# zsc/MOSS-TTSD

Measured on AMD Instinct MI355X. Metric: audio codec tokens/sec/node (decode, bf16, batch 32 @ 4k ctx), higher is better.
Workload: dtype bf16; 1 GPU; configs[2]: batch 32 synthetic dialogues/GPU, 4k-token KV context, top-k/top-p sampling on 8 channels, decode steps at full context; batch_per_gpu=32, context=4096, prompt=512, layers=28, hidden=2048, parallelism=dp1 (batch shard, no per-step collective)

## Files before the change

### moss-ttsd_amd/csrc/attn.hip

```cpp
#include "launch.h"
#include <algorithm>
#include <atomic>
#include <cstdlib>
#ifndef MTTS_PK_WAVES
#define MTTS_PK_WAVES 0
#endif
#if MTTS_PK_WAVES
#define PK_OCC(PK) __attribute__((amdgpu_waves_per_eu((PK) ? MTTS_PK_WAVES : 1, (PK) ? MTTS_PK_WAVES : 8)))
#else
#define PK_OCC(PK)
#endif

#include "seal.h"

__device__ bool seal_lane_k(const u32x4_t* __restrict__ raw, u32x4_t* __restrict__ pk, uint8_t* __restrict__ lds, int lane) {
    u32x4_t v[16];
#pragma unroll
    for (int j = 0; j < 16; ++j) v[j] = raw[j * 64];
    __builtin_amdgcn_wave_barrier();
    uint32_t* row = (uint32_t*)(lds + lane * 128);
#pragma unroll
    for (int j = 0; j < 16; ++j)
#pragma unroll
        for (int c = 0; c < 4; c += 2) {
// ... 128 lines not shown
    if (r < R) m = meta[r];
    unsigned long long todo = __ballot(m.seq >= 0 && (m.pos & 63) == 63);
    while (todo) {
        const int i = __ffsll((long long)todo) - 1;
        todo &= todo - 1;
        const int seq = __shfl(m.seq, i, 64), pos = __shfl(m.pos, i, 64);
        const int page = page_table[(size_t)seq * max_pages + (pos >> 6)];
        const size_t pi = (size_t)kvh * total_pages + page;
        const bool fit = wave ? seal_lane_v(vcache + layer * raw_layer + pi * (MTTS_PAGE * MTTS_HD / 8) + lane,
                                            vpack + layer * pk_layer + pi * (MTTS_PKU * 64) + lane, vlds, lane)
                              : seal_lane_k(kcache + layer * raw_layer + pi * (MTTS_PAGE * MTTS_HD / 8) + lane,
                                            kpack + layer * pk_layer + pi * (MTTS_PKU * 64) + lane, klds, lane);
        seal_count(fit, cnt, layer, wave, lane);
    }
}
__global__ __launch_bounds__(128) void kv_seal_all_kernel(const u32x4_t* __restrict__ kcache, const u32x4_t* __restrict__ vcache,
                                                          u32x4_t* __restrict__ kpack, u32x4_t* __restrict__ vpack, int total_pages,
                                                          size_t raw_layer, size_t pk_layer, unsigned long long* __restrict__ cnt) {
    __shared__ __attribute__((aligned(16))) uint8_t klds[8192 + 128];
    __shared__ __attribute__((aligned(16))) uint8_t vlds[8192 + 320];
    const int kvh = blockIdx.y, layer = blockIdx.z, wave = threadIdx.x >> 6, lane = threadIdx.x & 63;
    const size_t pi = (size_t)kvh * total_pages + blockIdx.x;
    const bool fit = wave ? seal_lane_v(vcache + layer * raw_layer + pi * (MTTS_PAGE * MTTS_HD / 8) + lane,
                                        vpack + layer * pk_layer + pi * (MTTS_PKU * 64) + lane, vlds, lane)
                          : seal_lane_k(kcache + layer * raw_layer + pi * (MTTS_PAGE * MTTS_HD / 8) + lane,
                                        kpack + layer * pk_layer + pi * (MTTS_PKU * 64) + lane, klds, lane);
    seal_count(fit, cnt, layer, wave, lane);
}
__global__ __launch_bounds__(64) void kv_seal_pages_kernel(const u32x4_t* __restrict__ raw, u32x4_t* __restrict__ pk, int as_k) {
    __shared__ __attribute__((aligned(16))) uint8_t klds[8192 + 320];
// ... 18 lines not shown
        n += 1;
        dk += __any(fk.w != 0u) ? 1 : 0;
        dv += __any(fv.w != 0u) ? 1 : 0;
    }
    if (lane == 0 && n) {
        atomicAdd(out + 0, n); atomicAdd(out + 1, dk); atomicAdd(out + 2, n); atomicAdd(out + 3, dv);
    }
}
void launch_kv_pack_count(const void* kpack, const void* vpack, const int32_t* page_table, const int32_t* complete, int B, int max_pages,
                          int total_pages, int nkv, int L, unsigned long long* out, hipStream_t st) {
    const size_t pk_layer = (size_t)total_pages * nkv * (MTTS_PKU * 64);
    hipLaunchKernelGGL(kv_pack_count_kernel, dim3(B, nkv, L), dim3(64), 0, st, (const u32x4_t*)kpack, (const u32x4_t*)vpack, page_table,
                       complete, max_pages, total_pages, pk_layer, out);
}
void launch_kv_seal_rows(const void* kcache, const void* vcache, void* kpack, void* vpack, const int32_t* page_table,
                         const RowMeta* meta, int R, int max_pages, int total_pages, int nkv, int L, unsigned long long* cnt, hipStream_t st) {
    const size_t raw_layer = (size_t)total_pages * nkv * (MTTS_PAGE * MTTS_HD / 8), pk_layer = (size_t)total_pages * nkv * (MTTS_PKU * 64);
    hipLaunchKernelGGL(kv_seal_scan_kernel, dim3((R + 63) / 64, nkv, L), dim3(128), 0, st, (const u32x4_t*)kcache, (const u32x4_t*)vcache,
                       (u32x4_t*)kpack, (u32x4_t*)vpack, page_table, meta, R, max_pages, total_pages, raw_layer, pk_layer, cnt);
}
void launch_kv_seal_all(const void* kcache, const void* vcache, void* kpack, void* vpack, int total_pages, int nkv, int L,
                        unsigned long long* cnt, hipStream_t st) {
    const size_t raw_layer = (size_t)total_pages * nkv * (MTTS_PAGE * MTTS_HD / 8), pk_layer = (size_t)total_pages * nkv * (MTTS_PKU * 64);
    hipLaunchKernelGGL(kv_seal_all_kernel, dim3(total_pages, nkv, L), dim3(128), 0, st, (const u32x4_t*)kcache, (const u32x4_t*)vcache,
                       (u32x4_t*)kpack, (u32x4_t*)vpack, total_pages, raw_layer, pk_layer, cnt);
}


__device__ __forceinline__ void fuse_reduce(const QkvFuse& f, int r, int col, int lane, float& a, float& b) {
    const size_t kstride = (size_t)MTTS_PFCAP * f.Npad;
    const float* p0 = f.partial + (size_t)r * f.Npad + col + lane;
    a = 0.f; b = 0.f;
    for (int k0 = 0; k0 < f.ksplit; k0 += 8) {
// ... 1068 lines not shown
```

### moss-ttsd_amd/csrc/engine.h

```cpp
#pragma once
#include <hip/hip_runtime.h>

#include <algorithm>
#include <cstdarg>
#include <cstdio>
#include <cstdlib>
#include <cstring>
#include <memory>
#include <string>
#include <vector>

#include "launch.h"
#include "runstate.h"
#include "stepplan.h"

static_assert(RUN_EINVAL == MTTS_EINVAL, "runstate.h reports with MTTS_EINVAL");

#define MTTS_LOCAL __attribute__((visibility("hidden")))
extern MTTS_LOCAL thread_local char g_err[512];
#define HIPCHK(x)                                                                          \
    do {                                                                                   \
        hipError_t _e = (x);                                                               \
        if (_e != hipSuccess) return fail(MTTS_EHIP, "%s: %s (%s:%d)", #x, hipGetErrorString(_e), __FILE__, __LINE__); \
    } while (0)
// ... 192 lines not shown

static inline bool rows_carry_adapters(const MttsEngine* e) {
    for (int b = 0; b < e->B; ++b)
        if (e->seq_adapter[b] >= 0) return true;
    return false;
}
static inline StepState step_state(const MttsEngine* e, int heads, int R, int pages_bound, bool lora) {
    StepState s;
    s.heads = heads; s.B = e->B; s.R = R; s.pages_bound = pages_bound; s.lora = lora;
    s.forced = e->has_forced; s.ch0_sampled = e->ch0_sampled != 0; s.scores_on = e->scores_on != 0; s.floors_on = e->floors_on != 0;
    s.bans_on = e->bans_on != 0;
    s.topk = e->topk_on;
    for (int k = 0; k < WSEAL_KINDS; ++k) s.wseal_on[k] = e->wseal_on[k] != 0;
    if (e->kpack) s.pack_k_on = e->pack_k_on.data();
    if (e->vpack) s.pack_v_on = e->pack_v_on.data();
    return s;
}
static inline StepPlan decode_plan(const MttsEngine* e, int pages_bound) {
    return plan_step(e->knobs, e->caps, step_state(e, 1, round_up(e->B, 32), pages_bound, rows_carry_adapters(e)));
}

static inline KvPack layer_pack(const MttsEngine* e, const StepPlan& plan, int n) {
    const LayerPlan& l = plan.layers[n];
    return KvPack{l.k_sealed ? (uint8_t*)e->kpack + e->pk_layer_stride * n : nullptr,
                  l.v_sealed ? (uint8_t*)e->vpack + e->pk_layer_stride * n : nullptr};
}
```

### moss-ttsd_amd/csrc/engine.hip

```cpp
#include "engine.h"
#include "staging.h"

#define FLUSH_STEPS 7
#define LINGER_STEPS 14
static inline int linger_bound(int B) { return 6 * B + 8; }

thread_local char g_err[512] = "";
int fail(int code, const char* fmt, ...) {
    va_list ap;
    va_start(ap, fmt);
    vsnprintf(g_err, sizeof(g_err), fmt, ap);
    va_end(ap);
    return code;
}

const char* mtts_last_error(void) { return g_err; }
int32_t mtts_version(void) { return 202; }

static auto ship_on(MttsEngine* e, hipStream_t st) {
    return [e, st](const PageEdits& ed) -> int {
        launch_set_pages(e->d_page_table, ed, st);
        HIPCHK(hipGetLastError());
        return 0;
    };
// ... 230 lines not shown
    }
    TRY(m.get(&e->d_seqs, MTTS_RCAP));
    TRY(m.get(&e->d_meta, MTTS_RCAP));
    TRY(m.get(&e->d_ls, 1));
    TRY(m.get_pinned(&e->h_ls, 1));
    TRY(m.get_pinned(&e->h_seqs, MTTS_RCAP));
    TRY(m.get(&e->d_decisions, MTTS_RCAP * 8));
    TRY(m.get(&e->d_cur, MTTS_RCAP * 8));
    TRY(m.get(&e->d_tf, MTTS_RCAP * 7 * 8));
    e->bm_words = (e->V0 + 31) / 32;
    TRY(m.get(&e->d_bitmaps, (size_t)MTTS_RCAP * 8 * e->bm_words));
    TRY(m.get(&e->d_scfg, 8));
    TRY(m.get(&e->d_floors, 8));
    TRY(m.get(&e->d_bancfg, 8));
    TRY(alloc_scratch(m, e->sscr, c->max_batch, e->V0));
    *out = holder.release();
    return MTTS_OK;
}

int32_t mtts_engine_destroy(MttsEngine* e) {
    if (!e) return MTTS_OK;
    hipSetDevice(e->device);
    hipDeviceSynchronize();
    e->graphs.clear();
    if (e->cap_stream) hipStreamDestroy(e->cap_stream);
    for (int w = 0; w < PROF_N; ++w) for (auto& pr : e->ev[w]) { hipEventDestroy(pr.first); hipEventDestroy(pr.second); }
    e->mem.free_all();
    const std::string err = e->mem.free_error;
    delete e;
    return err.empty() ? MTTS_OK : fail(MTTS_EHIP, "mtts_engine_destroy: %s", err.c_str());
// ... 339 lines not shown
    for (int i = 0; i < nphases; ++i) {
        hipEvent_t ev = nullptr;
        if (i < 2) prof_begin(e, i == 0 ? PROF_SCORES : PROF_PV, st, &ev);
        if (launch_attn(e->qbuf, kc, vc, e->d_page_table, d_meta, e->scores, e->stats, e->opart, e->attn_p, R,
                        pages_bound, e->max_pages, e->total_pages, e->nchunks_max, e->nq, e->nkv, scale,
                        fused ? &fz : nullptr, ph[i], st, pkp))
            return fail(MTTS_EINVAL, "attention group size not built");
        if (i < 2) prof_end(e, st, ev);
    }
    if (e->prof) {
        e->prof_bytes[PROF_SCORES] += kv_tokens_hint * e->nkv * MTTS_HD * 2;
        e->prof_bytes[PROF_PV] += kv_tokens_hint * e->nkv * MTTS_HD * 2;
    }
    return 0;
}
static void seal_completed_pages(MttsEngine* e, const RowMeta* d_meta, int R, hipStream_t st) {
    if (e->kpack)
        launch_kv_seal_rows(e->kcache, e->vcache, e->kpack, e->vpack, e->d_page_table, d_meta, R, e->max_pages, e->total_pages, e->nkv, e->L, e->d_seal_cnt, st);
}

static int forward_small(MttsEngine* e, const StepPlan& plan, const RowMeta* d_meta, int pages_bound, hipStream_t st, int64_t kv_tokens_hint) {
    const int H = e->H, I = e->I, nq = e->nq, Hp = round_up(H, 32), R = MTTS_MAXR;
    const float eps = e->cfg.rms_norm_eps;
    uint16_t* xa = (uint16_t*)e->x;
    uint16_t* xb = (uint16_t*)e->x2;
    SmallPro base{};
    base.rows = plan.B; base.eps = eps; base.slab_npad = Hp;
    for (int n = 0; n < e->L; ++n) {
        Layer& l = e->layers[n];
        SmallPro pq = base;
        pq.x_in = xa; pq.x_out = xb; pq.slabs = e->partial2; pq.ksplit = n ? e->p_d.ksplit : 0; pq.norm_w = (const uint16_t*)l.ln_in;
        launch_gemv_small(EPI_PARTIAL, PRO_NORM, e->p_qkv, l.wqkv, H, e->qkv_rows, e->qkv_rows, e->bufs.partial, nullptr, pq, st);
        TRY(attend_layer(e, plan, n, d_meta, R, pages_bound, e->p_qkv.ksplit, st, kv_tokens_hint));
        SmallPro po = base;
        po.opart = e->opart; po.meta = d_meta; po.nchunks_max = e->nchunks_max; po.nq = nq; po.pages_per_chunk = ATT_PB;
        launch_gemv_small(EPI_PARTIAL, PRO_COMBINE, e->p_o, l.wo, nq * MTTS_HD, Hp, Hp, e->partial2, nullptr, po, st);
        SmallPro pg = base;
        pg.x_in = xb; pg.x_out = xa; pg.slabs = e->partial2; pg.ksplit = e->p_o.ksplit; pg.norm_w = (const uint16_t*)l.ln_post;
        launch_gemv_small(EPI_SILU_RM, PRO_NORM, e->p_gu, l.wgu, H, 2 * I, 2 * I, nullptr, (uint16_t*)e->act_rm, pg, st);
        SmallPro pd = base;
        pd.xrows = (const uint16_t*)e->act_rm;
        launch_gemv_small(EPI_PARTIAL, PRO_ROWS, e->p_d, l.wd, I, Hp, Hp, e->partial2, nullptr, pd, st);
    }
    seal_completed_pages(e, d_meta, R, st);
    SmallPro ph = base;
    ph.x_in = xa; ph.x_out = nullptr; ph.slabs = e->partial2; ph.ksplit = e->p_d.ksplit; ph.norm_w = (const uint16_t*)e->final_norm;
    launch_gemv_small(EPI_BF16, PRO_NORM, e->p_h0, e->head0, H, e->V0_pad, e->V0, nullptr, (uint16_t*)e->logits0, ph, st);
    launch_gemv_small(EPI_BF16, PRO_NORM, e->p_h17, e->heads17, H, 7 * e->Vs_pad, 7 * e->Vs_pad, nullptr, (uint16_t*)e->logits17, ph, st);
    HIPCHK(hipGetLastError());
    return MTTS_OK;
}

static int run_gemm(int epi, bool tiled, int R, int ks, bool sealed, int head_form, const GemmPlan& p, const void* Ws, const void* Wp,
                    const void* Xp, int K, int Npad, int n_valid, float* partial, uint16_t* out, hipStream_t st) {
    const int mb = (R + 31) / 32;
    if (tiled) launch_gemm_tile(epi, R, ks, Wp, Xp, K, Npad, n_valid, partial, out, st);
    else if (!sealed) launch_gemm(epi, mb, p, Wp, Xp, K, Npad, n_valid, partial, out, st);
    else if (!launch_gemm_sealed(epi, mb, p, Ws, Wp, Xp, K, Npad, n_valid, partial, out, head_form, st))
        return fail(MTTS_ESTATE, "the plan asks for a sealed weight read that the launcher does not take (K %d, N %d, %d row tiles)", K, Npad, mb);
// ... 34 lines not shown
            TRY(run_gemm(EPI_PARTIAL, tiled, R, ks_o, false, 0, e->p_o, nullptr, l.wo, e->attn_p, QD, Hp, Hp, e->bufs.partial, nullptr, st));
            if (lora) delta(j_o, e->attn_p, ks_o);
            launch_resid_norm(e->bufs.partial, ks_o + ex, Hp, e->x, l.ln_post, e->xn, nullptr, d_meta, R, H, eps, st);
            TRY(run_gemm(gu_epi, tiled, R, 1, plan.sealed[WSEAL_GU], 0, e->p_gu, l.wgu_s, l.wgu, e->xn, H, 2 * I, 2 * I, gu_slab, (uint16_t*)e->act_p, st));
        }
        if (lora) {
            delta(j_gu, e->xn, 1);
            launch_swiglu_slabs(e->bufs.partial, e->bufs.partial + (size_t)MTTS_PFCAP * 2 * I, e->act_p, mb * 32, I, st);
        }
        TRY(run_gemm(EPI_PARTIAL, tiled, R, ks_d, plan.sealed[WSEAL_DOWN], 0, e->p_d, l.wd_s, l.wd, e->act_p, I, Hp, Hp, e->bufs.partial, nullptr, st));
        if (lora) delta(j_d, e->act_p, ks_d);
        const bool lastl = (n == e->L - 1);
        const void* nw = lastl ? e->final_norm : e->layers[n + 1].ln_in;
        launch_resid_norm(e->bufs.partial, ks_d + ex, Hp, e->x, nw, e->xn, lastl ? e->hlast : nullptr, d_meta, R, H, eps, st);
    }
    seal_completed_pages(e, d_meta, R, st);
    if (plan.heads) {
        const void* xin = e->xn;
        if (plan.heads == 2) {
            launch_pack_rows(e->hlast, e->xh, plan.B, H, plan.hmb, st);
            xin = e->xh;
        }
        const int hr = plan.hmb * 32, form = plan.head_persistent ? 1 : 0;
        TRY(run_gemm(EPI_BF16, false, hr, 0, plan.sealed[WSEAL_HEAD0], form, e->p_h0, e->head0_s, e->head0, xin, H, e->V0_pad, e->V0, nullptr, (uint16_t*)e->logits0, st));
        TRY(run_gemm(EPI_BF16, false, hr, 0, plan.sealed[WSEAL_HEADS], form, e->p_h17, e->heads17_s, e->heads17, xin, H, 7 * e->Vs_pad, 7 * e->Vs_pad, nullptr, (uint16_t*)e->logits17, st));
    }
    HIPCHK(hipGetLastError());
    return MTTS_OK;
}
static int forward_staged(MttsEngine* e, const int32_t* d_tokens, const RowMeta* d_meta, int R, int pages_bound, int heads, bool lora, hipStream_t st) {
    return forward_rows(e, plan_step(e->knobs, e->caps, step_state(e, heads, R, pages_bound, lora)), d_tokens, d_meta, pages_bound, st, 0);
// ... 1019 lines not shown
```

### moss-ttsd_amd/csrc/hooks.hip

```cpp
#include "engine.h"
#include "staging.h"

int32_t mtts_k_gemm_bf16(const void* w, const void* x, void* y, int32_t M, int32_t N, int32_t K, int32_t ksplit, void* stream) {
    if (!w || !x || !y || M < 1 || M > MTTS_PFCAP || K % 16 || N < 1) return fail(MTTS_EINVAL, "gemm: need 1<=M<=MTTS_PFCAP, K%%16==0");
    hipStream_t st = S(stream);
    int Npad = round_up(N, 32);
    void *wp = nullptr, *xp = nullptr;
    float* part = nullptr;
    GemmPlan p = mtts_plan_gemm(Npad, K, ksplit);
    p.depth = gemm_depth_env();
    DevBufs hb;
    TRY(hb.get((uint16_t**)&wp, (size_t)Npad * K));
    const bool tiled = M > MTTS_RCAP;
    const int ks = tiled ? (ksplit > 0 ? ksplit : mtts_tile_ksplit(Npad, K, M)) : p.ksplit;
    TRY(hb.get((uint16_t**)&xp, (size_t)MTTS_PFCAP * K));
    TRY(hb.get(&part, (size_t)ks * MTTS_PFCAP * Npad));
    launch_pack_weight(w, wp, N, K, Npad, 1, 0, st);
    const int tiles = (M + 31) / 32;
    launch_pack_rows(x, xp, M, K, tiles == 3 ? 4 : tiles, st);
    if (tiled) launch_gemm_tile(EPI_PARTIAL, M, ks, wp, xp, K, Npad, Npad, part, nullptr, st);
    else launch_gemm(EPI_PARTIAL, tiles, p, wp, xp, K, Npad, Npad, part, nullptr, st);
    launch_reduce_partial_bf16(part, y, ks, Npad, N, M, st);
    HIPCHK(hipGetLastError());
    HIPCHK(hipStreamSynchronize(st));
// ... 353 lines not shown
    HIPCHK(hipMemcpy(d, h, sizeof(h), hipMemcpyHostToDevice));
    MttsSamplerFloors* dfl = nullptr;
    if (floors) {
        MttsSamplerFloors hf[8];
        for (int i = 0; i < 8; ++i) hf[i] = *floors;
        PendingRun chk;
        TRY(chk.set_floors(hf));
        if (cfg->do_sample && (floors->min_p > 0.f || floors->epsilon_cutoff > 0.f || floors->eta_cutoff > 0.f)) {
            TRY(hb.get(&dfl, 8));
            HIPCHK(hipMemcpy(dfl, hf, sizeof(hf), hipMemcpyHostToDevice));
        }
    }
    SampleScratch sc;
    TRY(alloc_scratch(hb, sc, rows, vocab));
    sc.ban = (const uint32_t*)ban;
    if (dev_logp) {
        TRY(hb.get(&sc.slice_sum, (size_t)rows * SAMP_NS));
        TRY(hb.get(&sc.lp, (size_t)rows * 8));
    }
    launch_sample_single(logits, rows, vocab, (const uint32_t*)bitmap, (vocab + 31) / 32, d, mask_id, seed, step, channel, dec, err, sc,
                         full_cap_for(vocab), dev_logp ? 1 : 0, dfl, st);
    HIPCHK(hipGetLastError());
    HIPCHK(hipStreamSynchronize(st));
    std::vector<int32_t> hd((size_t)rows * 8);
    int32_t herr = 0;
    HIPCHK(hipMemcpy(hd.data(), dec, hd.size() * 4, hipMemcpyDeviceToHost));
    HIPCHK(hipMemcpy(&herr, err, 4, hipMemcpyDeviceToHost));
    std::vector<int32_t> outv(rows);
    for (int r = 0; r < rows; ++r) outv[r] = hd[(size_t)r * 8 + channel];
    HIPCHK(hipMemcpy(dev_tokens, outv.data(), rows * 4, hipMemcpyHostToDevice));
// ... 720 lines not shown
```

### moss-ttsd_amd/csrc/launch.h

```cpp
#pragma once
#include <type_traits>

#include "../../include/mtts.h"
#include "common.h"
#include "kvpool.h"

enum { EPI_PARTIAL = 0, EPI_BF16 = 1, EPI_SILU = 2,
       EPI_SILU_RM = 3 };
struct GemmPlan {
    int waves, ksplit, kt_per_split, kt_per_wave;
    int depth;
};
GemmPlan mtts_plan_gemm(int Npad, int K, int want_ksplit);
GemmPlan mtts_plan_gemm_forced(int Npad, int K, int ksplit, int waves);
void launch_gemm(int epi, int mb, const GemmPlan& p, const void* Wp, const void* Xp, int K, int Npad, int n_valid,
                 float* partial, uint16_t* out, hipStream_t st);
int mtts_gemm_form(int epi, int mb, const GemmPlan& p, int K, int Npad, int n_valid);
int mtts_tile_ksplit(int Npad, int K, int R);
void launch_gemm_tile(int epi, int R, int ksplit, const void* Wp, const void* Xp, int K, int Npad, int n_valid,
                      float* partial, uint16_t* out, hipStream_t st);
int mtts_small_lds_bytes(const GemmPlan& p, int K, int pro);
void launch_gemv_small(int epi, int pro, const GemmPlan& p, const void* Wp, int K, int Npad, int n_valid, float* partial,
                       uint16_t* out, const SmallPro& pr, hipStream_t st);
long long mtts_gemm_depth_launches();
// ... 34 lines not shown
void launch_unpack_rows(const void* packed, void* out, int R, int K, hipStream_t st);
void launch_bf16_round_check(unsigned long long* cnt2, hipStream_t st);

enum AttnPhase { ATTN_ALL = 0, ATTN_SCORES = 1, ATTN_PV = 2, ATTN_COMBINE = 3,
                 ATTN_ROW = 4,
                 ATTN_PF_SCORES = 11, ATTN_PF_PV = 12, ATTN_PF_COMBINE = 13 };
int launch_attn(const void* qbuf, void* kcache, void* vcache, const int32_t* page_table,
                const RowMeta* meta, void* scores, float* stats, float* opart, void* out_packed, int R,
                int pages_bound, int max_pages, int total_pages, int nchunks_max, int nq, int nkv, float scale,
                const QkvFuse* fuse, AttnPhase phase, hipStream_t st, const KvPack* pack = nullptr);
bool attn_row_fits(int G, const QkvFuse* fuse, const KvPack* pack, int pages_bound);
int attn_row_prepare();
int attn_row_lds_limit();
long long mtts_attn_row_launches();
void launch_kv_seal_rows(const void* kcache, const void* vcache, void* kpack, void* vpack, const int32_t* page_table,
                         const RowMeta* meta, int R, int max_pages, int total_pages, int nkv, int L, unsigned long long* cnt, hipStream_t st);
void launch_kv_seal_all(const void* kcache, const void* vcache, void* kpack, void* vpack, int total_pages, int nkv, int L,
                        unsigned long long* cnt, hipStream_t st);
void launch_kv_seal_pages(const void* raw, void* pk, int npages, int as_k, hipStream_t st);
void launch_kv_pack_count(const void* kpack, const void* vpack, const int32_t* page_table, const int32_t* complete, int B, int max_pages,
                          int total_pages, int nkv, int L, unsigned long long* out, hipStream_t st);

struct SeqState {
    int32_t nas;
    int32_t unfinished;
    int32_t kv_len;
    int32_t step;
    int32_t base_length;
    int32_t max_length;
    int32_t row_id;
    int32_t active;
// ... 18 lines not shown
struct SampleScratch {
    uint32_t* hist = nullptr;
    float* slice_val = nullptr;
    int32_t* slice_idx = nullptr;
    float* cand_val = nullptr;
    int32_t* cand_idx = nullptr;
    uint32_t* cand_n = nullptr;
    int32_t* overflow = nullptr;
    float* full_val = nullptr;
    int32_t* full_idx = nullptr;
    uint32_t* nuc_cnt = nullptr;
    unsigned long long* nuc_mass = nullptr;
    float* slice_sum = nullptr;
    float* lp = nullptr;
    const uint32_t* ban = nullptr;
};
void launch_sample(const void* logits0, const void* logits17, int V0, int Vs, int Vs_pad, const uint32_t* bitmaps,
                   int bm_words, const MttsSamplerCfg* cfgs, const LoopState* ls, const SeqState* seqs, uint64_t seed,
                   int32_t* decisions, int32_t* err, int B, const SampleScratch& sc, int ch0_sampled, int full_cap,
                   int emit_lp, const MttsSamplerFloors* floors , hipStream_t st);
void launch_sample_single(const void* logits, int rows, int vocab, const uint32_t* bitmap, int bm_words,
                          const MttsSamplerCfg* cfgs8, int mask_id, uint64_t seed, int step, int channel,
                          int32_t* decisions, int32_t* err, const SampleScratch& sc, int full_cap, int emit_lp,
                          const MttsSamplerFloors* floors8, hipStream_t st);
struct BanCfg { int32_t ngram, eos_below; };
void launch_ban(uint32_t* ban, const uint32_t* stat, int words, const BanCfg* cfgs, const int32_t* hist, int hist_cap,
                const int32_t* gen, int V0, int Vs, int eos, const LoopState* ls, const SeqState* seqs, int B, hipStream_t st);
void launch_ban_single(uint32_t* ban, const uint32_t* stat, const BanCfg* cfg1, const int32_t* hist, const int32_t* lens, int rows,
                       int cap, int vocab, int eos, hipStream_t st);
long long mtts_ban_launches();
// ... 73 lines not shown
```

### moss-ttsd_amd/csrc/sample_ctx.h

```cpp
#pragma once
#include "launch.h"

struct LogitsPtr { const void* p; int f32; };

struct SampleCtx {
    LogitsPtr lg;
    const uint32_t* bm;
    const uint32_t* ban;
    int V, mask_id, step, c;
    float penalty, temp;
    uint64_t seed;
    uint32_t row_id;
};

__device__ __forceinline__ bool sample_ctx(SampleCtx& x, int b, int c_in, const uint16_t* logits0,
                                           const uint16_t* logits17, int V0, int Vs, int Vs_pad,
                                           const uint32_t* bitmaps, int bm_words, const MttsSamplerCfg* cfgs,
                                           const LoopState* ls, const SeqState* seqs, int single_vocab, int single_mask,
                                           int single_step, int single_channel, const uint32_t* bans = nullptr) {
    if (single_vocab > 0) {
        x.c = single_channel; x.step = single_step; x.V = single_vocab; x.mask_id = single_mask;
        x.seed = 0; x.row_id = (uint32_t)b;
        x.lg = LogitsPtr{logits0 + (size_t)b * x.V, 0};
        x.bm = bitmaps ? bitmaps + (size_t)b * bm_words : nullptr;
        x.ban = bans ? bans + (size_t)b * ((x.V + 31) >> 5) : nullptr;
    } else {
        if (ls->done) return false;
        const SeqState sq = seqs[b];
// ... 21 lines not shown
```

### moss-ttsd_amd/csrc/sampler.hip

```cpp
#include "launch.h"
#include "sample_ctx.h"

__device__ __forceinline__ void philox4x32_10(uint32_t c0, uint32_t c1, uint32_t c2, uint32_t c3, uint32_t k0,
                                              uint32_t k1, uint32_t* out) {
#pragma unroll
    for (int i = 0; i < 10; ++i) {
        uint64_t p0 = (uint64_t)0xD2511F53u * c0;
        uint64_t p1 = (uint64_t)0xCD9E8D57u * c2;
        uint32_t n0 = (uint32_t)(p1 >> 32) ^ c1 ^ k0;
        uint32_t n1 = (uint32_t)p1;
        uint32_t n2 = (uint32_t)(p0 >> 32) ^ c3 ^ k1;
        uint32_t n3 = (uint32_t)p0;
        c0 = n0; c1 = n1; c2 = n2; c3 = n3;
        k0 += 0x9E3779B9u;
        k1 += 0xBB67AE85u;
    }
    out[0] = c0; out[1] = c1; out[2] = c2; out[3] = c3;
}

__device__ __forceinline__ uint32_t fkey(float f) {
    uint32_t u = __float_as_uint(f);
    return (u & 0x80000000u) ? ~u : (u | 0x80000000u);
}

__device__ __forceinline__ float proc_score(const SampleCtx& x, int i) {
    if (i == x.mask_id) return -INFINITY;
    if (x.ban && (x.ban[i >> 5] >> (i & 31)) & 1u) return -INFINITY;
    float s = x.lg.f32 ? ((const float*)x.lg.p)[i] : bf2f(((const uint16_t*)x.lg.p)[i]);
    if (x.penalty > 0.f && (x.bm[i >> 5] >> (i & 31)) & 1u) s = (s < 0.f) ? s * x.penalty : s / x.penalty;
    if (x.temp > 0.f) s = s / x.temp;
    return s;
}

#define SAMP_T 256

__device__ __forceinline__ void argmax_merge(float& bv, int& bi, float ov, int oi) {
    if (ov > bv || (ov == bv && oi < bi)) { bv = ov; bi = oi; }
}

__device__ __forceinline__ void block_argmax(float& bv, int& bi, float* shf, int* shi) {
#pragma unroll
    for (int o = 32; o > 0; o >>= 1) argmax_merge(bv, bi, __shfl_xor(bv, o, 64), __shfl_xor(bi, o, 64));
    const int wid = threadIdx.x >> 6, nw = blockDim.x >> 6;
    __syncthreads();
    if ((threadIdx.x & 63) == 0) { shf[wid] = bv; shi[wid] = bi; }
    __syncthreads();
    bv = shf[0]; bi = shi[0];
    for (int w = 1; w < nw; ++w) argmax_merge(bv, bi, shf[w], shi[w]);
    __syncthreads();
// ... 16 lines not shown
    total = tot;
    __syncthreads();
    return base + inc - v;
}

template <bool LP>
__global__ __launch_bounds__(SAMP_T) void sample_scan_kernel(
    const uint16_t* __restrict__ logits0, int V0, const uint32_t* __restrict__ bitmaps, int bm_words,
    const MttsSamplerCfg* __restrict__ cfgs, const LoopState* __restrict__ ls, const SeqState* __restrict__ seqs,
    SampleScratch sc, int single_vocab,
    int single_mask, int single_step, int single_channel) {
    __shared__ uint32_t hist[2048];
    __shared__ float shf[SAMP_T / 64];
    __shared__ int shi[SAMP_T / 64];
    __shared__ double shd[SAMP_T / 64];
    const int b = blockIdx.y, slice = blockIdx.x, tid = threadIdx.x;
    SampleCtx x;
    if (!sample_ctx(x, b, 0, logits0, nullptr, V0, 0, 0, bitmaps, bm_words, cfgs, ls, seqs, single_vocab, single_mask,
                    single_step, single_channel, sc.ban)) return;
    const MttsSamplerCfg cfg = cfgs[x.c];
    const bool want_hist = cfg.do_sample && cfg.top_k > 0 && cfg.top_k < x.V;
    for (int i = tid; i < 2048; i += SAMP_T) hist[i] = 0;
    __syncthreads();
    const int per = (x.V + SAMP_NS - 1) / SAMP_NS;
    const int i0 = slice * per, i1 = min(x.V, i0 + per);
    float bv = -INFINITY;
    int bi = 0x7fffffff;
    for (int i = i0 + tid; i < i1; i += SAMP_T) {
        float s = proc_score(x, i);
        argmax_merge(bv, bi, s, i);
        if (want_hist) atomicAdd(&hist[fkey(s) >> 21], 1u);
    }
    block_argmax(bv, bi, shf, shi);
    if (tid == 0) { sc.slice_val[b * SAMP_NS + slice] = bv; sc.slice_idx[b * SAMP_NS + slice] = bi; }
    if (LP && !cfg.do_sample) {
        float loc = 0.f;
        if (bv > -INFINITY)
            for (int i = i0 + tid; i < i1; i += SAMP_T) {
                const float s = proc_score(x, i);
                if (s > -INFINITY) loc += expf(s - bv);
            }
        double tot;
        (void)block_excl_scan<SAMP_T>((double)loc, shd, tot);
        if (tid == 0) sc.slice_sum[b * SAMP_NS + slice] = (float)tot;
    }
    if (want_hist)
        for (int i = tid; i < 2048; i += SAMP_T)
            if (hist[i]) atomicAdd(&sc.hist[(size_t)b * 2048 + i], hist[i]);
}

#define SAMP_FT 1024
#define NUC_BINS 2048
#define NUC_SCALE 35184372088832.0
typedef unsigned long long u64;

struct NucSel {
    uint32_t kmin;
    uint32_t kp;
    int idp;
};
__device__ __forceinline__ float unfkey(uint32_t k) { return __uint_as_float((k & 0x80000000u) ? (k & 0x7fffffffu) : ~k); }
__device__ __forceinline__ bool nuc_in(const NucSel& z, uint32_t key, int id) {
    return key > 0x007fffffu  && key >= z.kmin && (key > z.kp || (key == z.kp && id >= z.idp));
}
__device__ __forceinline__ int nuc_bin(uint32_t key, float lo) {
    const int b = (int)((unfkey(key) - lo) * ((float)(NUC_BINS - 1) / 32.0f));
    return min(max(b, 0), NUC_BINS - 1);
}

__device__ __forceinline__ u64 nuc_q(uint32_t key, float smax) { return (u64)((double)expf(unfkey(key) - smax) * NUC_SCALE); }

__device__ __forceinline__ void nuc_pass_a(const SampleCtx& x, float smax, float lo, uint32_t* __restrict__ keys,
                                           uint16_t* __restrict__ bins, unsigned int* cnt, u64* mass, int i0, int i1, int step) {
    for (int i = i0; i < i1; i += step) {
        const float s = proc_score(x, i) + 0.0f;
        const uint32_t key = fkey(s);
        keys[i] = key;
        if (s > -INFINITY) {
            const int d = nuc_bin(key, lo);
            bins[i] = (uint16_t)d;
            atomicAdd(&cnt[d], 1u);
            atomicAdd(&mass[d], nuc_q(key, smax));
        } else bins[i] = 0xffffu;
    }
}


__device__ __forceinline__ int topk_bin(const uint32_t* hist, uint32_t k, uint32_t* wsum, int* sh_b0) {
    const int tid = threadIdx.x, lane = tid & 63, wid = tid >> 6;
    const uint32_t* h = hist + tid * 8;
    uint32_t cnt[8], mine = 0;
#pragma unroll
    for (int j = 0; j < 8; ++j) { cnt[j] = h[j]; mine += cnt[j]; }
    uint32_t suf = mine;
#pragma unroll
    for (int o = 1; o < 64; o <<= 1) {
        uint32_t t = __shfl_down(suf, o, 64);
        if (lane + o < 64) suf += t;
    }
// ... 22 lines not shown
    __shared__ uint32_t wsum[SAMP_T / 64];
    __shared__ int sh_b0;
    const int b = blockIdx.y, slice = blockIdx.x, tid = threadIdx.x, lane = tid & 63, wid = tid >> 6;
    SampleCtx x;
    if (!sample_ctx(x, b, 0, logits0, nullptr, V0, 0, 0, bitmaps, bm_words, cfgs, ls, seqs, single_vocab, single_mask,
                    single_step, single_channel, sc.ban)) return;
    const MttsSamplerCfg cfg = cfgs[x.c];
    if (!cfg.do_sample) return;
    if (!(cfg.top_k > 0 && cfg.top_k < x.V) || cfg.top_k > SAMP_CAND) {
        __shared__ unsigned int a_cnt[2048];
        __shared__ unsigned long long a_mass[2048];
        float smax = sc.slice_val[b * SAMP_NS + (lane & (SAMP_NS - 1))];
        smax = wave_max(smax);
        for (int i = tid; i < 2048; i += SAMP_T) { a_cnt[i] = 0; a_mass[i] = 0; }
        __syncthreads();
        const int per = (x.V + SAMP_NS - 1) / SAMP_NS;
        const int i0 = slice * per, i1 = min(x.V, i0 + per);
        nuc_pass_a(x, smax, smax - 32.0f, (uint32_t*)(sc.full_idx + (size_t)b * full_cap), (uint16_t*)(sc.full_val + (size_t)b * full_cap),
                   a_cnt, a_mass, i0 + tid, i1, SAMP_T);
        __syncthreads();
        for (int i = tid; i < 2048; i += SAMP_T)
            if (a_cnt[i]) { atomicAdd(&sc.nuc_cnt[(size_t)b * 2048 + i], a_cnt[i]); atomicAdd(&sc.nuc_mass[(size_t)b * 2048 + i], a_mass[i]); }
        if (slice == 0 && tid == 0) { sc.cand_n[b] = SAMP_CAND + 1; sc.overflow[b] = 2; }
        return;
    }
    const int b0 = topk_bin(sc.hist + (size_t)b * 2048, (uint32_t)cfg.top_k, wsum, &sh_b0);
    const uint32_t ninf_key = fkey(-INFINITY);
    const int per = (x.V + SAMP_NS - 1) / SAMP_NS;
    const int i0 = slice * per, i1 = min(x.V, i0 + per);
    for (int i = i0 + tid; i < i1; i += SAMP_T) {
        float s = proc_score(x, i);
        uint32_t key = fkey(s);
        if ((int)(key >> 21) >= b0 && key > ninf_key) {
            uint32_t slot = atomicAdd(&sc.cand_n[b], 1u);
            if (slot < SAMP_CAND) { sc.cand_val[(size_t)b * SAMP_CAND + slot] = s; sc.cand_idx[(size_t)b * SAMP_CAND + slot] = i; }
        }
    }
}

template <int NT, bool FL>
__device__ int finish_sample(float* __restrict__ cval, int* __restrict__ cidx, int n, const MttsSamplerCfg& cfg, float smax,
                             uint32_t step, uint32_t b, uint32_t c, uint64_t seed, double* shd, int* sh_i, float* lp,
                             const MttsSamplerFloors& fl) {
    const int tid = threadIdx.x;
    int P = 1;
    while (P < n) P <<= 1;
    for (int i = n + tid; i < P; i += NT) { cval[i] = INFINITY; cidx[i] = 0x7fffffff; }
    __syncthreads();
    for (int kk = 2; kk <= P; kk <<= 1) {
        for (int j = kk >> 1; j > 0; j >>= 1) {
            for (int t = tid; t < P; t += NT) {
                int ixj = t ^ j;
// ... 779 lines not shown
```

### moss-ttsd_amd/csrc/stepplan.h

```cpp
#pragma once
#include <algorithm>
#include <cstdio>
#include <cstdlib>
#include <string>
#include <vector>

#include "shapes.h"

#define MTTS_FOLD_NORM_DEFAULT 0
struct StepKnobs {
    int small_rows = SMALL_RP;
    int fuse_qkv_max = 2560;
    int pack_min_work = 512;
    int attn_row = 1;
    int pf_mfma_pages = 0;
    int gemm_depth = 1;
    int fold_norm = MTTS_FOLD_NORM_DEFAULT;
    int w_seal = 1;
    int w_seal_head = 1;
    int kv_pack = 1;
    bool use_graphs = true;
};
static inline StepKnobs step_knobs_from_env() {
    StepKnobs k;
    const auto clamp = [](const char* g, int lo, int hi) { return std::min(std::max(atoi(g), lo), hi); };
    if (const char* g = getenv("MTTS_GRAPHS")) k.use_graphs = atoi(g) != 0;
    if (const char* g = getenv("MTTS_FUSE_QKV_MAX")) k.fuse_qkv_max = atoi(g);
    if (const char* g = getenv("MTTS_KV_PACK")) k.kv_pack = atoi(g);
    if (const char* g = getenv("MTTS_KV_PACK_MIN")) k.pack_min_work = atoi(g);
    if (const char* g = getenv("MTTS_PREFILL_MFMA_PAGES")) k.pf_mfma_pages = atoi(g);
    if (const char* g = getenv("MTTS_ATTN_ROW")) k.attn_row = clamp(g, 0, 2);
    if (const char* g = getenv("MTTS_SMALL_ROWS")) k.small_rows = clamp(g, 0, SMALL_RP);
    if (const char* g = getenv("MTTS_GEMM_DEPTH")) k.gemm_depth = atoi(g) != 0;
    if (const char* g = getenv("MTTS_FOLD_NORM")) k.fold_norm = atoi(g) != 0;
    if (const char* g = getenv("MTTS_W_SEAL")) k.w_seal = clamp(g, 0, 2);
    if (const char* g = getenv("MTTS_W_SEAL_HEAD")) k.w_seal_head = atoi(g) != 0;
    return k;
}
static inline int fold_norm_env() { return step_knobs_from_env().fold_norm; }
static inline int gemm_depth_env() { return step_knobs_from_env().gemm_depth; }

enum { GEMM_QKV = 0, GEMM_O = 1, GEMM_GU = 2, GEMM_DOWN = 3, GEMM_HEAD0 = 4, GEMM_HEADS = 5,
       GEMM_GU_SLAB = 6,
       GEMM_KINDS = 7 };
struct StepCaps {
    int G = 1, nkv = 1, L = 0;
    int n_cus = 0;
    bool f32 = false;
    bool small_fits = false;
    bool fold_shape = false;
    int row_lds_limit = 0;
    bool wseal_kind[WSEAL_KINDS] = {false, false, false, false};
    int gemm_form[GEMM_KINDS] = {0, 0, 0, 0, 0, 0, 0};
};

struct StepState {
    int heads = 1;
    int B = 0, R = 0;
    int pages_bound = 0;
    bool lora = false;
    bool forced = false, ch0_sampled = false, scores_on = false;
    bool floors_on = false;
    bool bans_on = false;
    int topk = 0;
    bool wseal_on[WSEAL_KINDS] = {false, false, false, false};
    const char* pack_k_on = nullptr;
    const char* pack_v_on = nullptr;
};

enum StepPath { PATH_F32 = 0, PATH_SMALL = 1, PATH_ROWS = 2 };
enum AttnForm { ATTN_FORM_ROW = 0,
                ATTN_FORM_TWO_PASS_FUSED = 1,
                ATTN_FORM_TWO_PASS_EPILOGUE = 2,
                ATTN_FORM_PREFILL_MFMA = 3 };
struct LayerPlan {
    AttnForm attn;
    bool k_sealed, v_sealed;
    bool operator==(const LayerPlan& o) const { return attn == o.attn && k_sealed == o.k_sealed && v_sealed == o.v_sealed; }
};
struct StepPlan {
    StepPath path = PATH_ROWS;
    int heads = 1, B = 0, R = 0;
    int mb = 1, hmb = 1;
    bool tiled = false;
    bool lora = false, fold = false;
    bool sealed[WSEAL_KINDS] = {false, false, false, false};
    bool head_persistent = false;
    std::vector<LayerPlan> layers;
    bool forced = false, ch0_sampled = false, scores_on = false, floors_on = false, bans_on = false;
    int topk = 0;
    int gemm_form[GEMM_KINDS] = {0, 0, 0, 0, 0, 0, 0};
    bool operator==(const StepPlan& o) const {
        return path == o.path && heads == o.heads && B == o.B && R == o.R && mb == o.mb && hmb == o.hmb && tiled == o.tiled &&
               lora == o.lora && fold == o.fold && std::equal(sealed, sealed + WSEAL_KINDS, o.sealed) &&
               head_persistent == o.head_persistent && layers == o.layers && forced == o.forced && ch0_sampled == o.ch0_sampled &&
               scores_on == o.scores_on && floors_on == o.floors_on && bans_on == o.bans_on && topk == o.topk && std::equal(gemm_form, gemm_form + GEMM_KINDS, o.gemm_form);
    }
    bool operator!=(const StepPlan& o) const { return !(*this == o); }
};

static inline bool attn_row_auto(int rows, int nkv, int n_cus) { return n_cus > 0 && rows * nkv >= n_cus; }

static inline StepPlan plan_step(const StepKnobs& k, const StepCaps& c, const StepState& s) {
    StepPlan p;
    const bool decode = s.heads == 1;
    p.heads = s.heads; p.B = s.B; p.R = s.R;
    if (decode) { p.forced = s.forced; p.ch0_sampled = s.ch0_sampled; p.scores_on = s.scores_on; p.floors_on = s.floors_on; p.bans_on = s.bans_on; p.topk = s.topk; }
    if (c.f32) { p.path = PATH_F32; return p; }
    const bool small = decode && !s.lora && s.B <= k.small_rows && c.small_fits;
    p.path = small ? PATH_SMALL : PATH_ROWS;
    const int work = s.B * s.pages_bound;
    const bool fused = decode && work <= k.fuse_qkv_max;
    const bool pack = decode && work >= k.pack_min_work;
    const bool row_shape = !small && decode && k.attn_row != 0 && (k.attn_row == 2 || attn_row_auto(s.B, c.nkv, c.n_cus));
    p.layers.resize(c.L);
    for (int n = 0; n < c.L; ++n) {
        LayerPlan& l = p.layers[n];
        l.k_sealed = pack && s.pack_k_on && s.pack_k_on[n];
        l.v_sealed = pack && s.pack_v_on && s.pack_v_on[n];
        const bool row = row_shape && l.k_sealed == l.v_sealed && attn_row_lds_bytes(c.G, l.k_sealed, s.pages_bound) <= c.row_lds_limit;
        l.attn = row ? ATTN_FORM_ROW : fused ? ATTN_FORM_TWO_PASS_FUSED :
                 (!decode && s.pages_bound >= k.pf_mfma_pages) ? ATTN_FORM_PREFILL_MFMA : ATTN_FORM_TWO_PASS_EPILOGUE;
    }
// ... 67 lines not shown
```

Before: 83740 codec_tokens/s.

## Skip KV seal launches on non-boundary steps and vectorize sampler score loads

The host planner now works out whether any live slot finishes a KV page this step. If none does, the seal kernel is skipped entirely, and when one does, a per-row seal kernel runs in place of the wave-scan kernel. Separately, the sampler's score passes now read bf16 logits in aligned 16-byte vectors, with several loads in flight per thread, and the log-prob sum is staged through LDS. Both paths sit behind env knobs, and the change adds plan-key variation that may cause extra graph captures.

```diff
diff --git a/moss-ttsd_amd/csrc/attn.hip b/moss-ttsd_amd/csrc/attn.hip
--- a/moss-ttsd_amd/csrc/attn.hip
+++ b/moss-ttsd_amd/csrc/attn.hip
@@ -166,6 +166,24 @@
         seal_count(fit, cnt, layer, wave, lane);
     }
 }
+__global__ __launch_bounds__(128) void kv_seal_row_kernel(const u32x4_t* __restrict__ kcache, const u32x4_t* __restrict__ vcache,
+                                                          u32x4_t* __restrict__ kpack, u32x4_t* __restrict__ vpack,
+                                                          const int32_t* __restrict__ page_table, const RowMeta* __restrict__ meta,
+                                                          int max_pages, int total_pages, size_t raw_layer, size_t pk_layer,
+                                                          unsigned long long* __restrict__ cnt) {
+    __shared__ __attribute__((aligned(16))) uint8_t klds[8192 + 128];
+    __shared__ __attribute__((aligned(16))) uint8_t vlds[8192 + 320];
+    const int kvh = blockIdx.y, layer = blockIdx.z, wave = threadIdx.x >> 6, lane = threadIdx.x & 63;
+    const RowMeta m = meta[blockIdx.x];
+    if (m.seq < 0 || (m.pos & 63) != 63) return;
+    const int page = page_table[(size_t)m.seq * max_pages + (m.pos >> 6)];
+    const size_t pi = (size_t)kvh * total_pages + page;
+    const bool fit = wave ? seal_lane_v(vcache + layer * raw_layer + pi * (MTTS_PAGE * MTTS_HD / 8) + lane,
+                                        vpack + layer * pk_layer + pi * (MTTS_PKU * 64) + lane, vlds, lane)
+                          : seal_lane_k(kcache + layer * raw_layer + pi * (MTTS_PAGE * MTTS_HD / 8) + lane,
+                                        kpack + layer * pk_layer + pi * (MTTS_PKU * 64) + lane, klds, lane);
+    seal_count(fit, cnt, layer, wave, lane);
+}
 __global__ __launch_bounds__(128) void kv_seal_all_kernel(const u32x4_t* __restrict__ kcache, const u32x4_t* __restrict__ vcache,
                                                           u32x4_t* __restrict__ kpack, u32x4_t* __restrict__ vpack, int total_pages,
                                                           size_t raw_layer, size_t pk_layer, unsigned long long* __restrict__ cnt) {
@@ -214,9 +232,13 @@
                        complete, max_pages, total_pages, pk_layer, out);
 }
 void launch_kv_seal_rows(const void* kcache, const void* vcache, void* kpack, void* vpack, const int32_t* page_table,
-                         const RowMeta* meta, int R, int max_pages, int total_pages, int nkv, int L, unsigned long long* cnt, hipStream_t st) {
+                         const RowMeta* meta, int R, int max_pages, int total_pages, int nkv, int L, unsigned long long* cnt, bool per_row,
+                         hipStream_t st) {
     const size_t raw_layer = (size_t)total_pages * nkv * (MTTS_PAGE * MTTS_HD / 8), pk_layer = (size_t)total_pages * nkv * (MTTS_PKU * 64);
-    hipLaunchKernelGGL(kv_seal_scan_kernel, dim3((R + 63) / 64, nkv, L), dim3(128), 0, st, (const u32x4_t*)kcache, (const u32x4_t*)vcache,
+    if (per_row)
+        hipLaunchKernelGGL(kv_seal_row_kernel, dim3(R, nkv, L), dim3(128), 0, st, (const u32x4_t*)kcache, (const u32x4_t*)vcache,
+                           (u32x4_t*)kpack, (u32x4_t*)vpack, page_table, meta, max_pages, total_pages, raw_layer, pk_layer, cnt);
+    else hipLaunchKernelGGL(kv_seal_scan_kernel, dim3((R + 63) / 64, nkv, L), dim3(128), 0, st, (const u32x4_t*)kcache, (const u32x4_t*)vcache,
                        (u32x4_t*)kpack, (u32x4_t*)vpack, page_table, meta, R, max_pages, total_pages, raw_layer, pk_layer, cnt);
 }
 void launch_kv_seal_all(const void* kcache, const void* vcache, void* kpack, void* vpack, int total_pages, int nkv, int L,
diff --git a/moss-ttsd_amd/csrc/engine.h b/moss-ttsd_amd/csrc/engine.h
--- a/moss-ttsd_amd/csrc/engine.h
+++ b/moss-ttsd_amd/csrc/engine.h
@@ -230,6 +230,10 @@
     for (int k = 0; k < WSEAL_KINDS; ++k) s.wseal_on[k] = e->wseal_on[k] != 0;
     if (e->kpack) s.pack_k_on = e->pack_k_on.data();
     if (e->vpack) s.pack_v_on = e->pack_v_on.data();
+    s.continuous = e->continuous;
+    if (heads == 1)
+        for (int b = 0; b < e->B && b < (int)e->n_real.size(); ++b)
+            if (e->slot_live[b] && (e->n_real[b] + e->steps_issued + 1) % MTTS_PAGE == 0) s.page_done = true;
     return s;
 }
 static inline StepPlan decode_plan(const MttsEngine* e, int pages_bound) {
diff --git a/moss-ttsd_amd/csrc/engine.hip b/moss-ttsd_amd/csrc/engine.hip
--- a/moss-ttsd_amd/csrc/engine.hip
+++ b/moss-ttsd_amd/csrc/engine.hip
@@ -268,6 +268,7 @@
     TRY(m.get(&e->d_floors, 8));
     TRY(m.get(&e->d_bancfg, 8));
     TRY(alloc_scratch(m, e->sscr, c->max_batch, e->V0));
+    e->sscr.vec = kn.sampler_vec;
     *out = holder.release();
     return MTTS_OK;
 }
@@ -637,9 +638,10 @@
     }
     return 0;
 }
-static void seal_completed_pages(MttsEngine* e, const RowMeta* d_meta, int R, hipStream_t st) {
-    if (e->kpack)
-        launch_kv_seal_rows(e->kcache, e->vcache, e->kpack, e->vpack, e->d_page_table, d_meta, R, e->max_pages, e->total_pages, e->nkv, e->L, e->d_seal_cnt, st);
+static void seal_completed_pages(MttsEngine* e, const StepPlan& plan, const RowMeta* d_meta, int R, hipStream_t st) {
+    if (e->kpack && plan.seal != SEAL_NONE)
+        launch_kv_seal_rows(e->kcache, e->vcache, e->kpack, e->vpack, e->d_page_table, d_meta, R, e->max_pages, e->total_pages, e->nkv, e->L, e->d_seal_cnt,
+                            plan.seal == SEAL_ROWS, st);
 }
 
 static int forward_small(MttsEngine* e, const StepPlan& plan, const RowMeta* d_meta, int pages_bound, hipStream_t st, int64_t kv_tokens_hint) {
@@ -665,7 +667,7 @@
         pd.xrows = (const uint16_t*)e->act_rm;
         launch_gemv_small(EPI_PARTIAL, PRO_ROWS, e->p_d, l.wd, I, Hp, Hp, e->partial2, nullptr, pd, st);
     }
-    seal_completed_pages(e, d_meta, R, st);
+    seal_completed_pages(e, plan, d_meta, R, st);
     SmallPro ph = base;
     ph.x_in = xa; ph.x_out = nullptr; ph.slabs = e->partial2; ph.ksplit = e->p_d.ksplit; ph.norm_w = (const uint16_t*)e->final_norm;
     launch_gemv_small(EPI_BF16, PRO_NORM, e->p_h0, e->head0, H, e->V0_pad, e->V0, nullptr, (uint16_t*)e->logits0, ph, st);
@@ -730,7 +732,7 @@
         const void* nw = lastl ? e->final_norm : e->layers[n + 1].ln_in;
         launch_resid_norm(e->bufs.partial, ks_d + ex, Hp, e->x, nw, e->xn, lastl ? e->hlast : nullptr, d_meta, R, H, eps, st);
     }
-    seal_completed_pages(e, d_meta, R, st);
+    seal_completed_pages(e, plan, d_meta, R, st);
     if (plan.heads) {
         const void* xin = e->xn;
         if (plan.heads == 2) {
diff --git a/moss-ttsd_amd/csrc/hooks.hip b/moss-ttsd_amd/csrc/hooks.hip
--- a/moss-ttsd_amd/csrc/hooks.hip
+++ b/moss-ttsd_amd/csrc/hooks.hip
@@ -391,6 +391,7 @@
     SampleScratch sc;
     TRY(alloc_scratch(hb, sc, rows, vocab));
     sc.ban = (const uint32_t*)ban;
+    sc.vec = sampler_vec_env();
     if (dev_logp) {
         TRY(hb.get(&sc.slice_sum, (size_t)rows * SAMP_NS));
         TRY(hb.get(&sc.lp, (size_t)rows * 8));
diff --git a/moss-ttsd_amd/csrc/launch.h b/moss-ttsd_amd/csrc/launch.h
--- a/moss-ttsd_amd/csrc/launch.h
+++ b/moss-ttsd_amd/csrc/launch.h
@@ -72,7 +72,8 @@
 int attn_row_lds_limit();
 long long mtts_attn_row_launches();
 void launch_kv_seal_rows(const void* kcache, const void* vcache, void* kpack, void* vpack, const int32_t* page_table,
-                         const RowMeta* meta, int R, int max_pages, int total_pages, int nkv, int L, unsigned long long* cnt, hipStream_t st);
+                         const RowMeta* meta, int R, int max_pages, int total_pages, int nkv, int L, unsigned long long* cnt,
+                         bool per_row , hipStream_t st);
 void launch_kv_seal_all(const void* kcache, const void* vcache, void* kpack, void* vpack, int total_pages, int nkv, int L,
                         unsigned long long* cnt, hipStream_t st);
 void launch_kv_seal_pages(const void* raw, void* pk, int npages, int as_k, hipStream_t st);
@@ -121,6 +122,7 @@
     float* slice_sum = nullptr;
     float* lp = nullptr;
     const uint32_t* ban = nullptr;
+    int vec = 1;
 };
 void launch_sample(const void* logits0, const void* logits17, int V0, int Vs, int Vs_pad, const uint32_t* bitmaps,
                    int bm_words, const MttsSamplerCfg* cfgs, const LoopState* ls, const SeqState* seqs, uint64_t seed,
diff --git a/moss-ttsd_amd/csrc/sample_ctx.h b/moss-ttsd_amd/csrc/sample_ctx.h
--- a/moss-ttsd_amd/csrc/sample_ctx.h
+++ b/moss-ttsd_amd/csrc/sample_ctx.h
@@ -12,6 +12,12 @@
     uint64_t seed;
     uint32_t row_id;
 };
+
+__device__ __forceinline__ void sample_slice(int V, int slice, int& i0, int& i1) {
+    const int per = (((V + SAMP_NS - 1) / SAMP_NS) + 7) & ~7;
+    i0 = slice * per;
+    i1 = min(V, i0 + per);
+}
 
 __device__ __forceinline__ bool sample_ctx(SampleCtx& x, int b, int c_in, const uint16_t* logits0,
                                            const uint16_t* logits17, int V0, int Vs, int Vs_pad,
diff --git a/moss-ttsd_amd/csrc/sampler.hip b/moss-ttsd_amd/csrc/sampler.hip
--- a/moss-ttsd_amd/csrc/sampler.hip
+++ b/moss-ttsd_amd/csrc/sampler.hip
@@ -32,7 +32,61 @@
     return s;
 }
 
+__device__ __forceinline__ uint32_t token_bits8(const uint32_t* __restrict__ w, int i) {
+    const int sh = i & 31;
+    uint32_t v = w[i >> 5] >> sh;
+    if (sh > 24) v |= w[(i >> 5) + 1] << (32 - sh);
+    return v & 0xffu;
+}
+__device__ __forceinline__ void proc_score8(const SampleCtx& x, int i, const u32x4_t& raw, float* __restrict__ s) {
+    const uint32_t banned = x.ban ? token_bits8(x.ban, i) : 0u;
+    const uint32_t seen = x.penalty > 0.f ? token_bits8(x.bm, i) : 0u;
+    const uint32_t w[4] = {raw.x, raw.y, raw.z, raw.w};
+#pragma unroll
+    for (int j = 0; j < 8; ++j) {
+        float v = bf2f((uint16_t)(w[j >> 1] >> (16 * (j & 1))));
+        if ((seen >> j) & 1u) v = (v < 0.f) ? v * x.penalty : v / x.penalty;
+        if (x.temp > 0.f) v = v / x.temp;
+        s[j] = (i + j == x.mask_id || ((banned >> j) & 1u)) ? -INFINITY : v;
+    }
+}
+
+template <int NT, int NV, typename F>
+__device__ __forceinline__ void for_scores(const SampleCtx& x, int i0, int i1, int vec, F f) {
+    const int tid = threadIdx.x;
+    if (i0 >= i1) return;
+    if (!vec || x.lg.f32) {
+        for (int i = i0 + tid; i < i1; i += NT) f(i, proc_score(x, i));
+        return;
+    }
+    const uint16_t* p = (const uint16_t*)x.lg.p;
+    const int head = (int)(((16u - ((uint32_t)(uintptr_t)(p + i0) & 15u)) & 15u) >> 1);
+    const int a0 = min(i0 + head, i1), ng = (i1 - a0) >> 3, a1 = a0 + 8 * ng;
+    for (int g0 = tid; g0 < ng; g0 += NT * NV) {
+        u32x4_t raw[NV];
+#pragma unroll
+        for (int u = 0; u < NV; ++u) {
+            const int g = g0 + u * NT;
+            if (g < ng) raw[u] = *(const u32x4_t*)(p + a0 + 8 * g);
+        }
+#pragma unroll
+        for (int u = 0; u < NV; ++u) {
+            const int g = g0 + u * NT;
+            if (g < ng) {
+                float s[8];
+                proc_score8(x, a0 + 8 * g, raw[u], s);
+#pragma unroll
+                for (int j = 0; j < 8; ++j) f(a0 + 8 * g + j, s[j]);
+            }
+        }
+    }
+    if (tid < a0 - i0) f(i0 + tid, proc_score(x, i0 + tid));
+    if (tid < i1 - a1) f(a1 + tid, proc_score(x, a1 + tid));
+}
+
 #define SAMP_T 256
+#define SAMP_NV 3
+#define SAMP_LP_STAGE 4864
 
 __device__ __forceinline__ void argmax_merge(float& bv, int& bi, float ov, int oi) {
     if (ov > bv || (ov == bv && oi < bi)) { bv = ov; bi = oi; }
@@ -79,6 +133,7 @@
     __shared__ float shf[SAMP_T / 64];
     __shared__ int shi[SAMP_T / 64];
     __shared__ double shd[SAMP_T / 64];
+    __shared__ float term[LP ? SAMP_LP_STAGE : 1];
     const int b = blockIdx.y, slice = blockIdx.x, tid = threadIdx.x;
     SampleCtx x;
     if (!sample_ctx(x, b, 0, logits0, nullptr, V0, 0, 0, bitmaps, bm_words, cfgs, ls, seqs, single_vocab, single_mask,
@@ -87,24 +142,29 @@
     const bool want_hist = cfg.do_sample && cfg.top_k > 0 && cfg.top_k < x.V;
     for (int i = tid; i < 2048; i += SAMP_T) hist[i] = 0;
     __syncthreads();
-    const int per = (x.V + SAMP_NS - 1) / SAMP_NS;
-    const int i0 = slice * per, i1 = min(x.V, i0 + per);
+    int i0, i1;
+    sample_slice(x.V, slice, i0, i1);
     float bv = -INFINITY;
     int bi = 0x7fffffff;
-    for (int i = i0 + tid; i < i1; i += SAMP_T) {
-        float s = proc_score(x, i);
+    for_scores<SAMP_T, SAMP_NV>(x, i0, i1, sc.vec, [&](int i, float s) {
         argmax_merge(bv, bi, s, i);
         if (want_hist) atomicAdd(&hist[fkey(s) >> 21], 1u);
-    }
+    });
     block_argmax(bv, bi, shf, shi);
     if (tid == 0) { sc.slice_val[b * SAMP_NS + slice] = bv; sc.slice_idx[b * SAMP_NS + slice] = bi; }
     if (LP && !cfg.do_sample) {
         float loc = 0.f;
-        if (bv > -INFINITY)
-            for (int i = i0 + tid; i < i1; i += SAMP_T) {
-                const float s = proc_score(x, i);
-                if (s > -INFINITY) loc += expf(s - bv);
-            }
+        if (bv > -INFINITY) {
+            if (sc.vec && !x.lg.f32 && i1 - i0 <= SAMP_LP_STAGE) {
+                for_scores<SAMP_T, SAMP_NV>(x, i0, i1, 1, [&](int i, float s) { term[i - i0] = s > -INFINITY ? expf(s - bv) : 0.f; });
+                __syncthreads();
+                for (int i = tid; i < i1 - i0; i += SAMP_T) loc += term[i];
+            } else
+                for (int i = i0 + tid; i < i1; i += SAMP_T) {
+                    const float s = proc_score(x, i);
+                    if (s > -INFINITY) loc += expf(s - bv);
+                }
+        }
         double tot;
         (void)block_excl_scan<SAMP_T>((double)loc, shd, tot);
         if (tid == 0) sc.slice_sum[b * SAMP_NS + slice] = (float)tot;
@@ -135,19 +195,21 @@
 
 __device__ __forceinline__ u64 nuc_q(uint32_t key, float smax) { return (u64)((double)expf(unfkey(key) - smax) * NUC_SCALE); }
 
+__device__ __forceinline__ void nuc_pass_a_token(int i, float ps, float smax, float lo, uint32_t* __restrict__ keys,
+                                                 uint16_t* __restrict__ bins, unsigned int* cnt, u64* mass) {
+    const float s = ps + 0.0f;
+    const uint32_t key = fkey(s);
+    keys[i] = key;
+    if (s > -INFINITY) {
+        const int d = nuc_bin(key, lo);
+        bins[i] = (uint16_t)d;
+        atomicAdd(&cnt[d], 1u);
+        atomicAdd(&mass[d], nuc_q(key, smax));
+    } else bins[i] = 0xffffu;
+}
 __device__ __forceinline__ void nuc_pass_a(const SampleCtx& x, float smax, float lo, uint32_t* __restrict__ keys,
                                            uint16_t* __restrict__ bins, unsigned int* cnt, u64* mass, int i0, int i1, int step) {
-    for (int i = i0; i < i1; i += step) {
-        const float s = proc_score(x, i) + 0.0f;
-        const uint32_t key = fkey(s);
-        keys[i] = key;
-        if (s > -INFINITY) {
-            const int d = nuc_bin(key, lo);
-            bins[i] = (uint16_t)d;
-            atomicAdd(&cnt[d], 1u);
-            atomicAdd(&mass[d], nuc_q(key, smax));
-        } else bins[i] = 0xffffu;
-    }
+    for (int i = i0; i < i1; i += step) nuc_pass_a_token(i, proc_score(x, i), smax, lo, keys, bins, cnt, mass);
 }
 
 
@@ -200,10 +262,11 @@
         smax = wave_max(smax);
         for (int i = tid; i < 2048; i += SAMP_T) { a_cnt[i] = 0; a_mass[i] = 0; }
         __syncthreads();
-        const int per = (x.V + SAMP_NS - 1) / SAMP_NS;
-        const int i0 = slice * per, i1 = min(x.V, i0 + per);
-        nuc_pass_a(x, smax, smax - 32.0f, (uint32_t*)(sc.full_idx + (size_t)b * full_cap), (uint16_t*)(sc.full_val + (size_t)b * full_cap),
-                   a_cnt, a_mass, i0 + tid, i1, SAMP_T);
+        int i0, i1;
+        sample_slice(x.V, slice, i0, i1);
+        uint32_t* keys = (uint32_t*)(sc.full_idx + (size_t)b * full_cap);
+        uint16_t* bins = (uint16_t*)(sc.full_val + (size_t)b * full_cap);
+        for_scores<SAMP_T, SAMP_NV>(x, i0, i1, sc.vec, [&](int i, float s) { nuc_pass_a_token(i, s, smax, smax - 32.0f, keys, bins, a_cnt, a_mass); });
         __syncthreads();
         for (int i = tid; i < 2048; i += SAMP_T)
             if (a_cnt[i]) { atomicAdd(&sc.nuc_cnt[(size_t)b * 2048 + i], a_cnt[i]); atomicAdd(&sc.nuc_mass[(size_t)b * 2048 + i], a_mass[i]); }
@@ -212,16 +275,15 @@
     }
     const int b0 = topk_bin(sc.hist + (size_t)b * 2048, (uint32_t)cfg.top_k, wsum, &sh_b0);
     const uint32_t ninf_key = fkey(-INFINITY);
-    const int per = (x.V + SAMP_NS - 1) / SAMP_NS;
-    const int i0 = slice * per, i1 = min(x.V, i0 + per);
-    for (int i = i0 + tid; i < i1; i += SAMP_T) {
-        float s = proc_score(x, i);
-        uint32_t key = fkey(s);
+    int i0, i1;
+    sample_slice(x.V, slice, i0, i1);
+    for_scores<SAMP_T, SAMP_NV>(x, i0, i1, sc.vec, [&](int i, float s) {
+        const uint32_t key = fkey(s);
         if ((int)(key >> 21) >= b0 && key > ninf_key) {
             uint32_t slot = atomicAdd(&sc.cand_n[b], 1u);
             if (slot < SAMP_CAND) { sc.cand_val[(size_t)b * SAMP_CAND + slot] = s; sc.cand_idx[(size_t)b * SAMP_CAND + slot] = i; }
         }
-    }
+    });
 }
 
 template <int NT, bool FL>
diff --git a/moss-ttsd_amd/csrc/stepplan.h b/moss-ttsd_amd/csrc/stepplan.h
--- a/moss-ttsd_amd/csrc/stepplan.h
+++ b/moss-ttsd_amd/csrc/stepplan.h
@@ -19,6 +19,8 @@
     int w_seal = 1;
     int w_seal_head = 1;
     int kv_pack = 1;
+    int seal_plan = 1;
+    int sampler_vec = 1;
     bool use_graphs = true;
 };
 static inline StepKnobs step_knobs_from_env() {
@@ -35,10 +37,13 @@
     if (const char* g = getenv("MTTS_FOLD_NORM")) k.fold_norm = atoi(g) != 0;
     if (const char* g = getenv("MTTS_W_SEAL")) k.w_seal = clamp(g, 0, 2);
     if (const char* g = getenv("MTTS_W_SEAL_HEAD")) k.w_seal_head = atoi(g) != 0;
+    if (const char* g = getenv("MTTS_SEAL_PLAN")) k.seal_plan = atoi(g) != 0;
+    if (const char* g = getenv("MTTS_SAMPLER_VEC")) k.sampler_vec = atoi(g) != 0;
     return k;
 }
 static inline int fold_norm_env() { return step_knobs_from_env().fold_norm; }
 static inline int gemm_depth_env() { return step_knobs_from_env().gemm_depth; }
+static inline int sampler_vec_env() { return step_knobs_from_env().sampler_vec; }
 
 enum { GEMM_QKV = 0, GEMM_O = 1, GEMM_GU = 2, GEMM_DOWN = 3, GEMM_HEAD0 = 4, GEMM_HEADS = 5,
        GEMM_GU_SLAB = 6,
@@ -66,6 +71,8 @@
     bool wseal_on[WSEAL_KINDS] = {false, false, false, false};
     const char* pack_k_on = nullptr;
     const char* pack_v_on = nullptr;
+    bool page_done = false;
+    bool continuous = false;
 };
 
 enum StepPath { PATH_F32 = 0, PATH_SMALL = 1, PATH_ROWS = 2 };
@@ -73,6 +80,9 @@
                 ATTN_FORM_TWO_PASS_FUSED = 1,
                 ATTN_FORM_TWO_PASS_EPILOGUE = 2,
                 ATTN_FORM_PREFILL_MFMA = 3 };
+enum SealForm { SEAL_NONE = 0,
+                SEAL_ROWS = 1,
+                SEAL_SCAN = 2 };
 struct LayerPlan {
     AttnForm attn;
     bool k_sealed, v_sealed;
@@ -86,6 +96,7 @@
     bool lora = false, fold = false;
     bool sealed[WSEAL_KINDS] = {false, false, false, false};
     bool head_persistent = false;
+    SealForm seal = SEAL_NONE;
     std::vector<LayerPlan> layers;
     bool forced = false, ch0_sampled = false, scores_on = false, floors_on = false, bans_on = false;
     int topk = 0;
@@ -93,7 +104,7 @@
     bool operator==(const StepPlan& o) const {
         return path == o.path && heads == o.heads && B == o.B && R == o.R && mb == o.mb && hmb == o.hmb && tiled == o.tiled &&
                lora == o.lora && fold == o.fold && std::equal(sealed, sealed + WSEAL_KINDS, o.sealed) &&
-               head_persistent == o.head_persistent && layers == o.layers && forced == o.forced && ch0_sampled == o.ch0_sampled &&
+               head_persistent == o.head_persistent && seal == o.seal && layers == o.layers && forced == o.forced && ch0_sampled == o.ch0_sampled &&
                scores_on == o.scores_on && floors_on == o.floors_on && bans_on == o.bans_on && topk == o.topk && std::equal(gemm_form, gemm_form + GEMM_KINDS, o.gemm_form);
     }
     bool operator!=(const StepPlan& o) const { return !(*this == o); }
@@ -107,6 +118,8 @@
     p.heads = s.heads; p.B = s.B; p.R = s.R;
     if (decode) { p.forced = s.forced; p.ch0_sampled = s.ch0_sampled; p.scores_on = s.scores_on; p.floors_on = s.floors_on; p.bans_on = s.bans_on; p.topk = s.topk; }
     if (c.f32) { p.path = PATH_F32; return p; }
+    if (s.pack_k_on || s.pack_v_on)
+        p.seal = (!decode || s.continuous || !k.seal_plan) ? SEAL_SCAN : s.page_done ? SEAL_ROWS : SEAL_NONE;
     const bool small = decode && !s.lora && s.B <= k.small_rows && c.small_fits;
     p.path = small ? PATH_SMALL : PATH_ROWS;
     const int work = s.B * s.pages_bound;
```

Measured after the change: 84240 codec_tokens/s (median of 6 runs). No clear change (+0.6%).
